# microsoft/StemGNN

Hardware: AMD Instinct MI355X
Metric: forecast-steps/sec (train) (higher is better)
Workload: dtype f32

## Files before the change

include/stemgnn_hip.h:

```cpp
#ifndef STEMGNN_HIP_H
#define STEMGNN_HIP_H

#include <stddef.h>
#include <stdint.h>

#ifdef __cplusplus
extern "C" {
#endif

#define SG_EINVAL (-10001)

#define SG_BLOCK_NPARAMS 33

const char* stemgnn_version(void);
int stemgnn_num_cus(void);

size_t stemgnn_table_floats(int W, int multi);
size_t stemgnn_packed_floats(int W, int multi);
size_t stemgnn_saved_floats(int B, int N, int W, int multi);
size_t stemgnn_scratch_floats(int B, int N, int W, int multi);
size_t stemgnn_gradpart_floats(int W, int multi, int nsplit);
size_t stemgnn_attn_saved_floats(int B, int N);
size_t stemgnn_attn_scratch_floats(int B, int N, int nchunk);
size_t stemgnn_scratch_offset_dG(int B, int N, int W, int multi);
// ... 58 lines not shown
int stemgnn_gru_bwd_overlap_ok(int B, int S, int Hd, int W);
size_t stemgnn_gru_bwd_ctl_words(int S);
int stemgnn_gru_bwd_rank2_begin(const float* dkey, const float* dquery, const float* wk, const float* wq, const float* x,
                                const float* w_hh, const float* h_ext, const float* reserve, int B, int S, int Hd, int W,
                                float* scratch, float* dw_ih, float* dw_hh, float* db_ih, float* db_hh, int* status,
                                unsigned* ctl, void* stream);
int stemgnn_gru_bwd_rank2_finish(const float* dkey, const float* dquery, const float* wk, const float* wq, const float* x,
                                 const float* w_hh, const float* h_ext, const float* reserve, int B, int S, int Hd, int W,
                                 float* scratch, float* dw_ih, float* dw_hh, float* db_ih, float* db_hh, int* status,
                                 unsigned* ctl, void* side_stream, void* stream);
int stemgnn_gru_bwd_recur(const float* dh_all, const float* x, const float* w_hh, const float* h_ext, const float* reserve,
                          int B, int S, int Hd, int W, float* scratch, int* status, void* stream);
int stemgnn_gru_bwd_rank2_recur(const float* dkey, float* dquery, int nchunk, const float* wk, const float* wq, const float* x,
                                const float* w_hh, const float* h_ext, const float* reserve, int B, int S, int Hd, int W,
                                float* scratch, int* status, void* stream);
int stemgnn_gru_input_grad(const float* scratch, const float* w_ih, int B, int S, int Hd, int W, float* dx, void* stream);

int stemgnn_block_pack(const float* const* params_host, const float* tables, float* packed,
                       int W, int multi, void* stream);
int stemgnn_block_pack_panels(const float* const* params_host, const float* tables, float* packed, int W, int multi,
                              void* stream);
int stemgnn_glu_fused_repack(float* packed, int W, int multi, void* stream);
int stemgnn_block_unpack_grads(const float* gradpart, int nsplit, const float* tables,
                               float* const* grads_host, int W, int multi, int has_backcast, void* stream);

int stemgnn_gft_fwd(const float* mul_L, const float* X, long xs_b, long xs_n, long xs_t,
                    float* G, int B, int N, int W, void* stream);
int stemgnn_gft_bwd(const float* mul_L, const float* X, long xs_b, long xs_n, long xs_t,
                    const float* dG, float* dX, float* dmul_L, int accumulate,
                    int B, int N, int W, void* stream);
int stemgnn_gft_bwd_dt2(const float* X0, long xs0_b, long xs0_n, long xs0_t, const float* dG0, const float* X1, long xs1_b,
                        long xs1_n, long xs1_t, const float* dG1, float* dmul_L, int B, int N, int W, void* stream);

int stemgnn_spectral_glu_fwd(const float* packed, float* saved, int B, int N, int W, int multi, void* stream);
int stemgnn_spectral_glu_bwd(const float* packed, const float* saved, float* scratch, float* gradpart,
                             int nsplit, int parts, int B, int N, int W, int multi, void* stream);
size_t stemgnn_glu_split_floats(int W, int multi, int splits);
int stemgnn_glu_split_panels(const float* packed, float* split, int W, int multi, int splits, void* stream);
int stemgnn_spectral_glu_fwd_split(const float* packed, const float* split, float* saved, int B, int N, int W, int multi,
                                   int splits, void* stream);
size_t stemgnn_glu_warm_saved_floats(int W, int multi);
int stemgnn_spectral_glu_fwd_warm(const float* packed, const float* split, float* saved, int B, int N, int W, int multi,
                                  int splits, void* stream);
int stemgnn_spectral_glu_dgrad_split(const float* packed, const float* split, const float* saved, float* scratch,
                                     int B, int N, int W, int multi, int splits, void* stream);
int stemgnn_glu_fused_bf16_ok(int W, int multi, int splits);

int stemgnn_igft_heads_fwd(const float* const* params_host, const float* packed, float* saved,
                           const float* X, long xs_b, long xs_n, long xs_t,
                           float* forecast, int accumulate, float* backcast,
                           int B, int N, int W, int multi, void* stream);
int stemgnn_igft_heads_bwd(const float* const* params_host, const float* packed, const float* saved,
                           const float* X, long xs_b, long xs_n, long xs_t,
                           const float* dforecast, const float* dbackcast, const float* backcast,
                           float* scratch, float* gradpart, int nsplit, int parts,
                           int B, int N, int W, int multi, void* stream);

int stemgnn_shortcut_dx(const float* scratch, const float* bs_w, float* dX, int B, int N, int W, int multi, void* stream);

int stemgnn_block_wgrad(const float* const* params_host, const float* packed, const float* saved,
                        const float* X, long xs_b, long xs_n, long xs_t, const float* dforecast, int has_bc,
                        float* scratch, float* gradpart, int nsplit, int cu_percent,
                        int B, int N, int W, int multi, void* stream);
int stemgnn_block_wgrad_split(const float* const* params_host, const float* packed, const float* saved,
                              const float* X, long xs_b, long xs_n, long xs_t, const float* dforecast, int has_bc,
                              float* scratch, float* gradpart, int nsplit, int cu_percent, int B, int N, int W,
// ... 74 lines not shown
```

stemgnn_amd/_lib.py:

```python
import ctypes
import os
from ctypes import POINTER, c_char_p, c_float, c_int, c_long, c_size_t, c_void_p

_HERE = os.path.dirname(os.path.abspath(__file__))
LIB_PATH = os.environ.get("STEMGNN_HIP_LIB", os.path.join(_HERE, "libstemgnn_hip.so"))
SG_BLOCK_NPARAMS = 33
SG_EINVAL = -10001
SG_PATH = {"glu_fwd_fused": 1, "glu_dgrad_fused": 2, "heads_fwd_fused": 4, "heads_bwd_fused": 8, "heads_bwd_16w": 16,
           "long_k": 32, "wgrad_fused": 64, "glu_wgrad_fused": 128}

_P = c_void_p
_PP = POINTER(c_void_p)

SIGNATURES = {
    "stemgnn_version": (c_char_p, []),
    "stemgnn_num_cus": (c_int, []),
    "stemgnn_table_floats": (c_size_t, [c_int, c_int]),
    "stemgnn_packed_floats": (c_size_t, [c_int, c_int]),
    "stemgnn_saved_floats": (c_size_t, [c_int, c_int, c_int, c_int]),
    "stemgnn_scratch_floats": (c_size_t, [c_int, c_int, c_int, c_int]),
    "stemgnn_scratch_offset_dG": (c_size_t, [c_int, c_int, c_int, c_int]),
    "stemgnn_gradpart_floats": (c_size_t, [c_int, c_int, c_int]),
    "stemgnn_attn_saved_floats": (c_size_t, [c_int, c_int]),
    "stemgnn_attn_scratch_floats": (c_size_t, [c_int, c_int, c_int]),
# ... 39 lines not shown
    "stemgnn_keyquery_wgrad": (c_int, [_P, _P, _P, _P, c_int, c_int, _P]),
    "stemgnn_attn_dquery_reduce": (c_int, [_P, c_int, c_int, c_int, _P, _P]),
    "stemgnn_keyquery_wgrad2": (c_int, [_P, _P, _P, _P, _P, c_int, c_int, _P]),
    "stemgnn_fc_tail_supported": (c_int, [c_int, c_int]),
    "stemgnn_fc_tail_scratch_floats": (c_size_t, [c_int, c_int, c_int, c_int]),
    "stemgnn_fc_tail_fwd": (c_int, [_P, _P, _P, _P, _P, c_int, c_int, c_int, c_int, _P, _P]),
    "stemgnn_fc_tail_bwd": (c_int, [_P, _P, _P, _P, _P, c_int, c_int, c_int, c_int, _P, _P, _P, _P, _P, _P, _P]),
    "stemgnn_fill_zero": (c_int, [_P, c_size_t, _P]),
    "stemgnn_rmsprop_step": (c_int, [_P, _P, _P, c_size_t, _P, c_float, c_float, c_int, c_float, _P]),
    "stemgnn_adam_step": (c_int, [_P, _P, _P, _P, c_size_t, _P, _P, c_float, c_float, c_float, c_int, c_float, _P]),
    "stemgnn_normalize_series": (c_int, [_P, _P, _P, c_int, _P, c_long, c_int, _P]),
    "stemgnn_window_gather": (c_int, [_P, _P, _P, _P, c_int, c_int, c_int, c_int, c_long, _P, _P]),
    "stemgnn_window_gather_queue": (c_int, [_P, _P, _P, _P, _P, c_int, c_int, c_int, c_int, c_long, _P, _P]),
    "stemgnn_mse_scratch_floats": (c_size_t, []),
    "stemgnn_mse_fwd": (c_int, [_P, _P, c_size_t, _P, _P, _P, _P]),
    "stemgnn_mse_bwd": (c_int, [_P, _P, c_size_t, _P, _P, _P]),
    "stemgnn_roll_window": (c_int, [_P, _P, _P, _P, c_int, c_int, c_int, c_int, c_int, c_int, _P]),
    "stemgnn_forecast_store": (c_int, [_P, _P, _P, _P, _P, c_int, c_int, c_int, c_long, _P]),
    "stemgnn_eval_scratch_doubles": (c_size_t, [c_long, c_int, c_int]),
    "stemgnn_eval_out_doubles": (c_size_t, [c_int, c_int]),
    "stemgnn_eval_metrics": (c_int, [_P, _P, _P, _P, c_long, c_int, c_int, _P, _P, _P]),
    "stemgnn_block_pack": (c_int, [_PP, _P, _P, c_int, c_int, _P]),
    "stemgnn_block_pack_panels": (c_int, [_PP, _P, _P, c_int, c_int, _P]),
    "stemgnn_block_unpack_grads": (c_int, [_P, c_int, _P, _PP, c_int, c_int, c_int, _P]),
    "stemgnn_gft_fwd": (c_int, [_P, _P, c_long, c_long, c_long, _P, c_int, c_int, c_int, _P]),
    "stemgnn_gft_bwd": (c_int, [_P, _P, c_long, c_long, c_long, _P, _P, _P, c_int, c_int, c_int, c_int, _P]),
    "stemgnn_gft_bwd_dt2": (c_int, [_P, c_long, c_long, c_long, _P, _P, c_long, c_long, c_long, _P, _P, c_int, c_int, c_int, _P]),
    "stemgnn_spectral_glu_fwd": (c_int, [_P, _P, c_int, c_int, c_int, c_int, _P]),
    "stemgnn_spectral_glu_bwd": (c_int, [_P, _P, _P, _P, c_int, c_int, c_int, c_int, c_int, c_int, _P]),
    "stemgnn_glu_split_floats": (c_size_t, [c_int, c_int, c_int]),
    "stemgnn_glu_split_panels": (c_int, [_P, _P, c_int, c_int, c_int, _P]),
    "stemgnn_glu_fused_bf16_ok": (c_int, [c_int, c_int, c_int]),
    "stemgnn_block_paths": (c_int, [c_int, c_int, c_int, c_int, c_int]),
    "stemgnn_spectral_glu_fwd_split": (c_int, [_P, _P, _P, c_int, c_int, c_int, c_int, c_int, _P]),
    "stemgnn_glu_warm_saved_floats": (c_size_t, [c_int, c_int]),
    "stemgnn_spectral_glu_fwd_warm": (c_int, [_P, _P, _P, c_int, c_int, c_int, c_int, c_int, _P]),
    "stemgnn_spectral_glu_dgrad_split": (c_int, [_P, _P, _P, _P, c_int, c_int, c_int, c_int, c_int, _P]),
    "stemgnn_igft_heads_fwd": (c_int, [_PP, _P, _P, _P, c_long, c_long, c_long, _P, c_int, _P,
                                       c_int, c_int, c_int, c_int, _P]),
    "stemgnn_igft_heads_bwd": (c_int, [_PP, _P, _P, _P, c_long, c_long, c_long, _P, _P, _P, _P, _P, c_int, c_int,
                                       c_int, c_int, c_int, c_int, _P]),
    "stemgnn_fc_tail_train_scratch_floats": (c_size_t, [c_int, c_int, c_int, c_int]),
    "stemgnn_fc_tail_train": (c_int, [_P, _P, _P, _P, _P, _P, c_int, c_int, c_int, c_int, _P, _P, _P, _P, _P, _P, _P, _P,
                                      _P, _P]),
    "stemgnn_fc_tail_train_rows": (c_int, [_P, _P, _P, _P, _P, _P, c_int, c_int, c_int, c_int, _P, _P, _P, _P]),
    "stemgnn_fc_tail_train_finish": (c_int, [_P, c_int, c_int, c_int, c_int, _P, _P, _P, _P, _P, _P, _P]),
    "stemgnn_infer_workspace_floats": (c_size_t, [c_int, c_int, c_int, c_int]),
    "stemgnn_infer_workspace_split_floats": (c_size_t, [c_int, c_int, c_int, c_int, c_int]),
    "stemgnn_gru_fwd_infer": (c_int, [_P, _P, _P, _P, _P, c_int, c_int, c_int, c_int, _P, _P, _P, _P]),
    "stemgnn_spectral_glu_fwd_infer": (c_int, [_P, _P, c_size_t, c_int, c_int, c_int, c_int, _P]),
    "stemgnn_spectral_glu_fwd_split_infer": (c_int, [_P, _P, _P, c_size_t, c_int, c_int, c_int, c_int, c_int, _P]),
    "stemgnn_igft_heads_fwd_infer": (c_int, [_PP, _P, _P, c_size_t, _P, c_long, c_long, c_long, _P, c_int, _P,
                                             c_int, c_int, c_int, c_int, _P]),
    "stemgnn_block_wgrad": (c_int, [_PP, _P, _P, _P, c_long, c_long, c_long, _P, c_int, _P, _P, c_int, c_int,
                                    c_int, c_int, c_int, c_int, _P]),
    "stemgnn_block_wgrad_split": (c_int, [_PP, _P, _P, _P, c_long, c_long, c_long, _P, c_int, _P, _P, c_int, c_int,
                                          c_int, c_int, c_int, c_int, c_int, _P]),
}

_lib = None


class StemGNNHipError(RuntimeError):
    pass


# ... 30 lines not shown
```

stemgnn_amd/csrc/block.hip:

```cpp
#include <hip/hip_runtime.h>

#include "../../include/stemgnn_hip.h"
#include "devattr.h"
#include "gemm2.h"
#include "gemm2s.h"
#include "gemm_core.h"
#include "layout.h"
#include "reduce.h"
#include "wgrad.h"
#include "heads.h"
#include "glu_fused.h"
#include "glu_fused_bf16.h"

#define SG_TRY(e)                                \
  do {                                           \
    hipError_t _e = (e);                         \
    if (_e != hipSuccess) return -(int)_e;       \
  } while (0)

__device__ __forceinline__ float sg_sigmoid(float v) { return __frcp_rn(1.f + __expf(-v)); }

struct SgDiv {
  unsigned d, magic;
  __device__ __forceinline__ int div(int x) const { return d == 1u ? x : (int)__umulhi((unsigned)x, magic); }
// ... 414 lines not shown
    const int w = z / S;
    const int n = nb[w];
    const int kb = k / rdiv[w], kr = k - kb * rdiv[w];
    const float v = pb[w][kb * sb[w] + kr * sn[w] + (j < n ? j : n - 1) * st[w]];
    return j < n ? v : 1.f;
  }
  __device__ void epi(int z, int i, int j, float v) const {
    const int w = z / S, s = z - w * S;
    part[w][((size_t)s * Mw[w] + i) * ldp[w] + j] = v;
  }
};

constexpr int SG_LONG_K = 640;
constexpr int SG_WG_MAX_TILES = 256;
static inline bool wg_tiles_fit(WgGemm* q, int n) { return wg_tile_index(q, n) <= SG_WG_MAX_TILES; }
static inline int split_chunk(int M, int S) { return ((M + S - 1) / S + 15) & ~15; }

extern "C" int stemgnn_gft_fwd(const float* mul_L, const float* X, long xs_b, long xs_n, long xs_t,
                               float* G, int B, int N, int W, void* stream) {
  if (!mul_L || !X || !G || B <= 0 || N <= 0 || W <= 0) return SG_EINVAL;
  if (!sg_div_ok(3L * N + 64, N) || !sg_div_ok((long)B * W + 64, W)) return SG_EINVAL;
  GftFwdOp op{mul_L + (size_t)N * N, XView{X, xs_b, xs_n, xs_t, N}, G, B, N, W, sg_div(N), sg_div(W)};
  hipStream_t st = (hipStream_t)stream;
  if (N <= 512) {
    if (xs_n == 1) SG_TRY((sg_launch_gemm<GftFwdOp, 32, 32, true, true, false, 128, true>(op, 3 * N, B * W, 1, st)));
    else SG_TRY((sg_launch_gemm<GftFwdOp, 32, 32, true, false, false, 128, true>(op, 3 * N, B * W, 1, st)));
    return 0;
  }
  if (xs_n == 1) SG_TRY((sg_launch_gemm<GftFwdOp, 32, 64, true, true, false, 64, true>(op, 3 * N, B * W, 1, st)));
  else SG_TRY((sg_launch_gemm<GftFwdOp, 32, 64, true, false, false, 64, true>(op, 3 * N, B * W, 1, st)));
  return 0;
}

extern "C" int stemgnn_gft_bwd(const float* mul_L, const float* X, long xs_b, long xs_n, long xs_t,
                               const float* dG, float* dX, float* dmul_L, int accumulate,
                               int B, int N, int W, void* stream) {
  if (!mul_L || !X || !dG || (!dmul_L && !dX) || B <= 0 || N <= 0 || W <= 0) return SG_EINVAL;
  hipStream_t st = (hipStream_t)stream;
  const bool bk128 = N <= 512;
  if (!sg_div_ok(3L * N + 128, N) || !sg_div_ok((long)B * W + 128, W)) return SG_EINVAL;
  if (dX) {
    GftBwdDxOp op{mul_L + (size_t)N * N, dG, dX, B, N, W, (size_t)B * N * 3 * W, sg_div(N), sg_div(W)};
    if (bk128) SG_TRY((sg_launch_gemm<GftBwdDxOp, 32, 32, false, false, false, 128, true>(op, N, B * W, 1, st)));
    else SG_TRY((sg_launch_gemm<GftBwdDxOp, 32, 32, false, false, false, 64, true>(op, N, B * W, 1, st)));
  }
  if (!dmul_L) return 0;
  GftBwdDtOp op{dG, XView{X, xs_b, xs_n, xs_t, N}, dmul_L + (size_t)N * N, B, N, W, accumulate, (size_t)B * N * 3 * W, sg_div(N),
                sg_div(W)};
  if (bk128) {
    if (xs_t == 1) SG_TRY((sg_launch_gemm<GftBwdDtOp, 32, 32, true, true, false, 128, true>(op, 3 * N, N, 1, st)));
    else SG_TRY((sg_launch_gemm<GftBwdDtOp, 32, 32, true, false, false, 128, true>(op, 3 * N, N, 1, st)));
    return 0;
  }
  if (xs_t == 1) SG_TRY((sg_launch_gemm<GftBwdDtOp, 32, 32, true, true, false, 64, true>(op, 3 * N, N, 1, st)));
  else SG_TRY((sg_launch_gemm<GftBwdDtOp, 32, 32, true, false, false, 64, true>(op, 3 * N, N, 1, st)));
  return 0;
}

extern "C" int stemgnn_gft_bwd_dt2(const float* X0, long xs0_b, long xs0_n, long xs0_t, const float* dG0, const float* X1,
                                   long xs1_b, long xs1_n, long xs1_t, const float* dG1, float* dmul_L, int B, int N, int W,
                                   void* stream) {
  if (!X0 || !dG0 || !X1 || !dG1 || !dmul_L || B <= 0 || N <= 0 || W <= 0) return SG_EINVAL;
  hipStream_t st = (hipStream_t)stream;
  if (!sg_div_ok(3L * N + 128, N) || !sg_div_ok(2L * B * W + 128, W)) return SG_EINVAL;
  GftBwdDt2Op op{{dG0, dG1}, {XView{X0, xs0_b, xs0_n, xs0_t, N}, XView{X1, xs1_b, xs1_n, xs1_t, N}}, dmul_L + (size_t)N * N,
                 B, N, W, (size_t)B * N * 3 * W, sg_div(N), sg_div(W)};
  if (N <= 512) SG_TRY((sg_launch_gemm<GftBwdDt2Op, 32, 32, true, false, false, 128, true>(op, 3 * N, N, 1, st)));
  else SG_TRY((sg_launch_gemm<GftBwdDt2Op, 32, 32, true, false, false, 64, true>(op, 3 * N, N, 1, st)));
  return 0;
}

struct GluFwdBufs {
  const float* G;
  float* out[2][3];
  float* gate[2][3];
};
static GluFwdBufs glu_bufs_saved(const SgDims& d, float* saved) {
  const SgSavedLayout S = sg_saved_layout(d);
  GluFwdBufs b;
  b.G = saved + S.G;
  for (int r = 0; r < 2; ++r)
    for (int l = 0; l < 3; ++l) { b.out[r][l] = saved + S.out[r][l]; b.gate[r][l] = saved + S.gate[r][l]; }
  return b;
}
static GluFwdBufs glu_bufs_infer(const SgDims& d, float* ws, bool pp) {
  const SgInferLayout I = sg_infer_layout(d, pp);
  GluFwdBufs b;
  b.G = ws + I.G;
  for (int r = 0; r < 2; ++r) {
    b.out[r][0] = pp ? ws + I.pp[r][0] : nullptr;
    b.out[r][1] = pp ? ws + I.pp[r][1] : nullptr;
    b.out[r][2] = ws + I.out2[r];
    for (int l = 0; l < 3; ++l) b.gate[r][l] = nullptr;
  }
  return b;
}
template <bool INF>
static int glu_fwd_layers(const SgDims& d, const float* packed, const unsigned short* const* fpl, int splits,
                          const GluFwdBufs& bf, hipStream_t st) {
  const SgPackedLayout P = sg_packed_layout(d);
  using Epi = GluFwdEpiT<!INF>;
  for (int l = 0; l < 3; ++l) {
// ... 837 lines not shown
```

stemgnn_amd/csrc/front.hip:

```cpp
#include <hip/hip_runtime.h>
#include <stdlib.h>
#include <stdint.h>

#include "../../include/stemgnn_hip.h"
#include "dq_reduce.h"
#include "gemm_core.h"
#include "layout.h"

#define SG_TRY(e)                                \
  do {                                           \
    hipError_t _e = (e);                         \
    if (_e != hipSuccess) return -(int)_e;       \
  } while (0)

constexpr int ATTN_NBC = 8;

__device__ __forceinline__ void sg_philox4(uint64_t seed, uint64_t offset, uint64_t idx, uint32_t (&w)[4]) {
  uint32_t c0 = (uint32_t)idx, c1 = (uint32_t)(idx >> 32), c2 = (uint32_t)offset, c3 = (uint32_t)(offset >> 32);
  uint32_t k0 = (uint32_t)seed, k1 = (uint32_t)(seed >> 32);
#pragma unroll
  for (int r = 0; r < 10; ++r) {
    const uint32_t hi0 = __umulhi(0xD2511F53u, c0), lo0 = 0xD2511F53u * c0;
    const uint32_t hi1 = __umulhi(0xCD9E8D57u, c2), lo1 = 0xCD9E8D57u * c2;
    c0 = hi1 ^ c1 ^ k0; c1 = lo1; c2 = hi0 ^ c3 ^ k1; c3 = lo0;
// ... 691 lines not shown
  if (!seed || !used || seed == used) return SG_EINVAL;
  hipLaunchKernelGGL(sg_dropout_seed_next_kernel, dim3(1), dim3(64), 0, (hipStream_t)stream, seed, used);
  SG_TRY(hipGetLastError());
  return 0;
}

extern "C" int stemgnn_dropout_mask(float drop_p, const uint64_t* seed, int B, int N, float* mask, void* stream) {
  if (!seed || !mask || B <= 0 || N <= 0) return SG_EINVAL;
  const size_t n = (size_t)B * N * N;
  hipLaunchKernelGGL(sg_dropout_mask_kernel, dim3((unsigned)((n + 255) / 256)), dim3(256), 0, (hipStream_t)stream,
                     drop_p, seed, n, N, mask);
  SG_TRY(hipGetLastError());
  return 0;
}

extern "C" int stemgnn_cheb_fwd(float* mul_L, int N, void* stream) {
  if (!mul_L || N <= 0) return SG_EINVAL;
  hipStream_t st = (hipStream_t)stream;
  const size_t nn = (size_t)N * N;
  float* L = mul_L + nn;
  ChebFwdOp op2{L, L, mul_L + 2 * nn, N, 0};
  if (N <= 512) {
    SG_TRY((sg_launch_gemm<ChebFwdOp, 32, 32, true, false, false, 128, true>(op2, N, N, 1, st)));
    ChebFwdOp op3b{L, mul_L + 2 * nn, mul_L + 3 * nn, N, 1};
    SG_TRY((sg_launch_gemm<ChebFwdOp, 32, 32, true, false, false, 128, true>(op3b, N, N, 1, st)));
    return 0;
  }
  SG_TRY((sg_launch_gemm<ChebFwdOp, 32, 32, true, false, false, 64, true>(op2, N, N, 1, st)));
  ChebFwdOp op3{L, mul_L + 2 * nn, mul_L + 3 * nn, N, 1};
  SG_TRY((sg_launch_gemm<ChebFwdOp, 32, 32, true, false, false, 64, true>(op3, N, N, 1, st)));
  return 0;
}

extern "C" int stemgnn_cheb_bwd(const float* mul_L, const float* dmul_L, float* dL, float* scratch, int N,
                                void* stream) {
  if (!mul_L || !dmul_L || !dL || !scratch || N <= 0) return SG_EINVAL;
  hipStream_t st = (hipStream_t)stream;
  const size_t nn = (size_t)N * N;
  float* dLp = scratch;
  float* dT2p = scratch + nn;
  ChebBwd1Op op1{mul_L + nn, mul_L + 2 * nn, dmul_L + nn, dmul_L + 2 * nn, dmul_L + 3 * nn, dLp, dT2p, N};
  if (N <= 512) {
    SG_TRY((sg_launch_gemm<ChebBwd1Op, 32, 32, true, true, false, 128, true>(op1, N, N, 2, st)));
    ChebBwd2Op op2b{mul_L + nn, dT2p, dLp, dL, N};
    SG_TRY((sg_launch_gemm<ChebBwd2Op, 32, 32, true, true, false, 128, true>(op2b, N, N, 1, st)));
    return 0;
  }
  SG_TRY((sg_launch_gemm<ChebBwd1Op, 32, 32, true, true, false, 64, true>(op1, N, N, 2, st)));
  ChebBwd2Op op2{mul_L + nn, dT2p, dLp, dL, N};
  SG_TRY((sg_launch_gemm<ChebBwd2Op, 32, 32, true, true, false, 64, true>(op2, N, N, 1, st)));
  return 0;
}
```

stemgnn_amd/csrc/gemm_core.h:

```cpp
#pragma once
#include <hip/hip_runtime.h>

typedef float sg_f32x4 __attribute__((ext_vector_type(4)));
#ifndef SG_CHAIN_PRIO
#define SG_CHAIN_PRIO 3
#endif

template <class Op, int BM, int BN, bool A_KFAST, bool B_KFAST, bool PAIR, int BK = 16, bool TWO_LEVEL = false>
__global__ __launch_bounds__(256) void sg_gemm_f32(const Op op) {
  static_assert(BK % 16 == 0, "BK");
  constexpr int TM = BM / 32;
  constexpr int TN = BN / 32;
  constexpr int SA = BM + (A_KFAST ? 17 : 16);
  constexpr int SB = BN + (B_KFAST ? 17 : 16);
  constexpr int RA = BM * BK / 256;
  constexpr int RB = BN * BK / 256;
  static_assert(BM % 32 == 0 && BN % 32 == 0, "tile");
  static_assert(!PAIR || (TN % 2 == 0), "PAIR needs an even number of 16-col tiles per wave");

  __builtin_amdgcn_s_setprio(SG_CHAIN_PRIO);
  __shared__ float lds[BK * SA + BK * SB];
  float* As = lds;
  float* Bs = lds + BK * SA;

  const int z = blockIdx.z;
  int M, N, K0, K1;
  if (!op.setup(z, M, N, K0, K1)) return;
  const int m0 = blockIdx.x * BM;
  const int n0 = blockIdx.y * BN;
  if (m0 >= M || n0 >= N) return;

  const int tid = threadIdx.x;
  const int lane = tid & 63;
  const int wave = tid >> 6;
// ... 91 lines not shown
  }

#pragma unroll
  for (int i = 0; i < TM; ++i) {
#pragma unroll
    for (int reg = 0; reg < 4; ++reg) {
      const int gi = m0 + wm * (BM / 2) + i * 16 + fk * 4 + reg;
      if (gi >= M) continue;
      if constexpr (PAIR) {
#pragma unroll
        for (int j = 0; j < TN; j += 2) {
          const int q0 = n0 + wn * (BN / 2) + j * 16;
          const int c = (q0 >> 1) + fi;
          if (q0 < N) op.epi2(z, gi, c, acc[i][j][reg], acc[i][j + 1][reg]);
        }
      } else {
#pragma unroll
        for (int j = 0; j < TN; ++j) {
          const int gj = n0 + wn * (BN / 2) + j * 16 + fi;
          if (gj < N) op.epi(z, gi, gj, acc[i][j][reg]);
        }
      }
    }
  }
}

template <class Op, int BM, int BN, bool A_KFAST, bool B_KFAST, bool PAIR, int BK = 16, bool TWO_LEVEL = false>
static inline hipError_t sg_launch_gemm(const Op& op, int maxM, int maxN, int nz, hipStream_t stream) {
  dim3 grid((maxM + BM - 1) / BM, (maxN + BN - 1) / BN, nz);
  if (grid.x == 0 || grid.y == 0 || grid.z == 0) return hipSuccess;
  hipLaunchKernelGGL((sg_gemm_f32<Op, BM, BN, A_KFAST, B_KFAST, PAIR, BK, TWO_LEVEL>), grid, dim3(256), 0, stream, op);
  return hipGetLastError();
}
```

stemgnn_amd/ops.py:

```python
import os
import weakref

import torch

from . import _lib

_NSPLIT = 32
_side_streams = {}


def _side_stream(device, index=0):
    key = (str(device), index)
    st = _side_streams.get(key)
    if st is None:
        st = torch.cuda.Stream(device=device)
        _side_streams[key] = st
    return st


def fresh_side_stream(device, index=0):
    _side_streams.pop((str(device), index), None)
    return _side_stream(device, index)


class HotPathState:

    def __init__(self):
        self.direct = False
        self.overlap = False
        self.prepacked = None
        self.preseed = None
        self.fork_event = None
        self.pending = None
        self.exact_group = None
        self.gru_front_live = False
        self.dh_factors = None
        self.block_grads_hook = None
        self.gru_ctl = None
        self.gru_ctl_zeroed = False
        self.warm_saved = None
        self.tail_finish = None
        self.side_probe = None
        _states.add(self)

    def set(self, direct=True, overlap=False):
        self.direct = bool(direct)
        self.overlap = bool(direct) and bool(overlap)
        return self

    def join(self):
        item, self.pending = self.pending, None
        if item is not None:
            side, keep = item
            torch.cuda.current_stream().wait_stream(side)
            del keep

    def reset(self):
        for item in (self.prepacked, self.pending):
            if item is not None:
                try:
                    (item[1] if item is self.prepacked else item[0]).synchronize()
                except RuntimeError:
                    pass
        self.prepacked = None
        self.preseed = None
        self.fork_event = None
        self.pending = None
        self.dh_factors = None
        self.gru_ctl_zeroed = False
        self.tail_finish = None


_states = weakref.WeakSet()
_NO_STATE = None
# ... 15 lines not shown


def _all_reduce_mean(t, group_world):
    group, world = group_world[0], group_world[1]
    fn = group_world[2] if len(group_world) > 2 else None
    if fn is not None:
        fn(t)
    else:
        import torch.distributed as dist
        dist.all_reduce(t, op=dist.ReduceOp.SUM, group=group)
    t.div_(world)


def set_direct_grad(model, flag=True, overlap=False):
    return model.hot_state.set(flag, overlap)


_NCHUNK = 16


def _wg_cu(which, B, N):
    if which == 0:
        return 90
    if N > 512:
        return 50
    lib = _lib.load()
    cus = lib.stemgnn_num_cus()
    busy = lib.stemgnn_gru_bwd_cus(B, N)
    return max(10, min(100, (cus - busy) * 100 // cus))


def _stream():
    return torch.cuda.current_stream().cuda_stream


def glu_splits():
    v = os.environ.get("STEMGNN_DTYPE", "f32").lower()
    if v in ("f32", "fp32", ""):
        return 0
    if v == "bf16x3":
        return 3
    if v == "bf16x2":
        return 2
    raise _lib.StemGNNHipError(f"STEMGNN_DTYPE={v!r}: expected f32, bf16x3 or bf16x2")


def _pack_block(lib, parr, tables, pk, W, multi, splits, stream):
    if splits:
        _lib.check(lib.stemgnn_block_pack_panels(parr, tables.data_ptr(), pk.data_ptr(), W, multi, stream), "block_pack_panels")
    else:
        _lib.check(lib.stemgnn_block_pack(parr, tables.data_ptr(), pk.data_ptr(), W, multi, stream), "block_pack")


def _split_panels(lib, pk, W, multi, splits, device, stream):
    sp = torch.empty(lib.stemgnn_glu_split_floats(W, multi, splits), device=device, dtype=torch.float32)
    _lib.check(lib.stemgnn_glu_split_panels(pk.data_ptr(), sp.data_ptr(), W, multi, splits, stream), "glu_split_panels")
    return sp


def _require_gpu(t, name):
    if not t.is_cuda:
        raise _lib.StemGNNHipError(
            f"{name} is on {t.device}: stemgnn_amd runs only on a HIP device (no CPU fallback)")
    if t.dtype != torch.float32:
        raise _lib.StemGNNHipError(f"{name} must be float32, got {t.dtype}")

# ... 593 lines not shown
            has_bc = s == 0
            garr = _lib.ptr_array(grads[s])
            keep.append((parr, garr))

            def heads(stream):
                _lib.check(lib.stemgnn_igft_heads_bwd(
                    parr, packed[s].data_ptr(), saved[s].data_ptr(), X.data_ptr(), sb, sn, stt, dfsum.data_ptr(),
                    dbackcast.data_ptr() if has_bc else None, backcast.data_ptr() if has_bc else None,
                    scratch.data_ptr(), gradpart.data_ptr(), nsplit, 1, B, N, W, multi, stream), "igft_heads_bwd")

            def glu(stream):
                if splits:
                    _lib.check(lib.stemgnn_spectral_glu_dgrad_split(
                        packed[s].data_ptr(), split[s].data_ptr(), saved[s].data_ptr(), scratch.data_ptr(),
                        B, N, W, multi, splits, stream), "spectral_glu_dgrad_split")
                    return
                _lib.check(lib.stemgnn_spectral_glu_bwd(
                    packed[s].data_ptr(), saved[s].data_ptr(), scratch.data_ptr(), gradpart.data_ptr(), nsplit, 1,
                    B, N, W, multi, stream), "spectral_glu_bwd")

            def wgrad(stream, cu_percent):
                _lib.check(lib.stemgnn_block_wgrad_split(
                    parr, packed[s].data_ptr(), saved[s].data_ptr(), X.data_ptr(), sb, sn, stt, dfsum.data_ptr(),
                    int(has_bc), scratch.data_ptr(), gradpart.data_ptr(), nsplit, cu_percent, B, N, W, multi,
                    2 if splits == 2 and os.environ.get("STEMGNN_WGRAD_BF16", "1") != "0" else 0, stream), "block_wgrad")

            def unpack(stream):
                _lib.check(lib.stemgnn_block_unpack_grads(
                    gradpart.data_ptr(), nsplit, tables.data_ptr(), garr, W, multi, int(has_bc), stream),
                    "block_unpack_grads")

            return heads, glu, wgrad, unpack

        dt1 = None
        for s in (1, 0):
            scratch = bufs[s][0]
            dG = scratch[off_dG:]
            X, sb, sn, stt = xviews[s]
            heads, glu, wgrad, unpack = stage_fns(s)
            heads(st)
            glu(st)
            if not overlap:
                if live[s]:
                    wgrad(st, 100)
                    unpack(st)
                _lib.check(lib.stemgnn_gft_bwd(
                    mul_L.data_ptr(), X.data_ptr(), sb, sn, stt, dG.data_ptr(),
                    dbackcast.data_ptr() if s == 1 else None, dmul_L.data_ptr(), int(s == 0), B, N, W, st), "gft_bwd")
            elif s == 1:
                _lib.check(lib.stemgnn_gft_bwd(mul_L.data_ptr(), X.data_ptr(), sb, sn, stt, dG.data_ptr(),
                                               dbackcast.data_ptr(), None, 0, B, N, W, st), "gft_bwd dX")
                dt1 = (X, sb, sn, stt, dG)
            else:
                fork = torch.cuda.Event()
                fork.record(main)
                X1, sb1, sn1, stt1, dG1 = dt1
                _lib.check(lib.stemgnn_gft_bwd_dt2(X.data_ptr(), sb, sn, stt, dG.data_ptr(), X1.data_ptr(), sb1, sn1, stt1,
                                                   dG1.data_ptr(), dmul_L.data_ptr(), B, N, W, st), "gft_bwd_dt2")
                side.wait_event(fork)
                with torch.cuda.stream(side):
                    sst = side.cuda_stream
                    for ss in (0, 1):
                        if not live[ss]:
                            continue
                        _h, _g, w2, u2 = (heads, glu, wgrad, unpack) if ss == 0 else stage_fns(1)
                        w2(sst, _wg_cu(ss, B, N))
                        u2(sst)
                        if state.side_probe is not None:
                            state.side_probe.append(lambda stream, w2=w2, pc=_wg_cu(ss, B, N): w2(stream, pc))
                            state.side_probe.append(u2)
                    if tail_finish is not None:
                        tail_finish(sst)
                        keep.append(tail_finish)
                        if state.side_probe is not None:
                            state.side_probe.append(tail_finish)
                    if state.block_grads_hook is not None:
                        state.block_grads_hook()
                keep.append(bufs)
        dX0 = None
        if nig[1]:
            X, sb, sn, stt = xviews[0]
            dX0 = torch.empty(B, N, W, device=dev, dtype=f32)
            _lib.check(lib.stemgnn_gft_bwd(mul_L.data_ptr(), X.data_ptr(), sb, sn, stt, scratch0[off_dG:].data_ptr(),
                                           dX0.data_ptr(), None, 0, B, N, W, st), "gft_bwd dX")
            _lib.check(lib.stemgnn_shortcut_dx(scratch0.data_ptr(), blocks[0][7].data_ptr(), dX0.data_ptr(), B, N, W, multi, st),
                       "shortcut_dx")
        if overlap:
            state.pending = (side, (keep, packed, saved, split, backcast, dfsum, dbackcast))
        dL = torch.empty(N, N, device=dev, dtype=f32)
        cheb_scratch = torch.empty(2 * N * N, device=dev, dtype=f32)
        _lib.check(lib.stemgnn_cheb_bwd(mul_L.data_ptr(), dmul_L.data_ptr(), dL.data_ptr(), cheb_scratch.data_ptr(),
                                        N, st), "cheb_bwd")
        factored = ctx.factored and ctx.needs_input_grad[0] and bool(lib.stemgnn_gru_bwd_rank2_ok(B, N))
        dh = torch.empty(1, device=dev, dtype=f32).expand(N, B, N) if factored else torch.empty_like(h)
        kq_direct = kq_live and state.direct and wk.grad is not None and wq.grad is not None
        if kq_live:
            dwk = wk.grad if kq_direct else torch.empty_like(wk)
            dwq = wq.grad if kq_direct else torch.empty_like(wq)
        elif factored:
            dwk = dwq = None
        else:
            dwk, dwq = torch.empty(2, N, device=dev, dtype=f32)
        _ptr = lambda t: None if t is None else t.data_ptr()
        attn_scratch = torch.empty(lib.stemgnn_attn_scratch_floats(B, N, _NCHUNK), device=dev, dtype=f32)
        use_drop = training and drop_p > 0.0
        exact = state.exact_group
        follower = bool(overlap and ctx.factored and state.gru_ctl_zeroed and lib.stemgnn_gru_bwd_overlap_ok(B, N, N, W))
        dq_parts = bool(factored and overlap and kq_direct and not follower)
        if not kq_live:
            dq_parts = bool(factored and not follower)
        for part in ((3,) if exact is None else (1, 2)):
            _lib.check(lib.stemgnn_attn_laplacian_bwd(
                dL.data_ptr(), h.data_ptr(), wk.data_ptr(), wq.data_ptr(), alpha, drop_p, int(training),
                seed.data_ptr() if use_drop else None, B, N, attn_saved.data_ptr(), attn_scratch.data_ptr(), _NCHUNK,
                None if factored else dh.data_ptr(), _ptr(dwk), _ptr(dwq),
                part | ((4 | (8 if dq_parts else 0)) if factored and part != 1 else 0), st), "attn_laplacian_bwd")
            if exact is not None and part == 1:
                _all_reduce_mean(attn_scratch[:N * N], exact)
        if factored:
            after = None
            if overlap and kq_direct:
                kq_ready = torch.cuda.Event()
                kq_ready.record(main)
                pend, hh, kdwk, kdwq = state.pending, h, dwk, dwq
                dq2 = torch.empty(B, N, device=dev, dtype=f32) if dq_parts else None
# ... 256 lines not shown
```

Measured before the change: 84620.

## Add split-K GEMM with workspace for graph backward products

```diff
diff --git a/include/stemgnn_hip.h b/include/stemgnn_hip.h
--- a/include/stemgnn_hip.h
+++ b/include/stemgnn_hip.h
@@ -114,6 +114,23 @@
 int stemgnn_gft_bwd_dt2(const float* X0, long xs0_b, long xs0_n, long xs0_t, const float* dG0, const float* X1, long xs1_b,
                         long xs1_n, long xs1_t, const float* dG1, float* dmul_L, int B, int N, int W, void* stream);
 
+#define SG_GP_GFT_DX  0
+#define SG_GP_GFT_DT  1
+#define SG_GP_GFT_DT2 2
+#define SG_GP_CHEB1   3
+#define SG_GP_CHEB2   4
+size_t stemgnn_graph_ws_floats(int B, int N, int W);
+int stemgnn_graph_splitk(int product, int B, int N, int W);
+int stemgnn_graph_ktiles(int product, int B, int N, int W);
+int stemgnn_gft_bwd_ws(const float* mul_L, const float* X, long xs_b, long xs_n, long xs_t,
+                       const float* dG, float* dX, float* dmul_L, int accumulate,
+                       int B, int N, int W, float* ws, int splitk, void* stream);
+int stemgnn_gft_bwd_dt2_ws(const float* X0, long xs0_b, long xs0_n, long xs0_t, const float* dG0, const float* X1, long xs1_b,
+                           long xs1_n, long xs1_t, const float* dG1, float* dmul_L, int B, int N, int W, float* ws, int splitk,
+                           void* stream);
+int stemgnn_cheb_bwd_ws(const float* mul_L, const float* dmul_L, float* dL, float* scratch, int B, int N, int W, float* ws,
+                        int splitk, void* stream);
+
 int stemgnn_spectral_glu_fwd(const float* packed, float* saved, int B, int N, int W, int multi, void* stream);
 int stemgnn_spectral_glu_bwd(const float* packed, const float* saved, float* scratch, float* gradpart,
                              int nsplit, int parts, int B, int N, int W, int multi, void* stream);
diff --git a/stemgnn_amd/_lib.py b/stemgnn_amd/_lib.py
--- a/stemgnn_amd/_lib.py
+++ b/stemgnn_amd/_lib.py
@@ -95,6 +95,13 @@
     "stemgnn_glu_split_panels": (c_int, [_P, _P, c_int, c_int, c_int, _P]),
     "stemgnn_glu_fused_bf16_ok": (c_int, [c_int, c_int, c_int]),
     "stemgnn_block_paths": (c_int, [c_int, c_int, c_int, c_int, c_int]),
+    "stemgnn_graph_ws_floats": (c_size_t, [c_int, c_int, c_int]),
+    "stemgnn_graph_splitk": (c_int, [c_int, c_int, c_int, c_int]),
+    "stemgnn_graph_ktiles": (c_int, [c_int, c_int, c_int, c_int]),
+    "stemgnn_gft_bwd_ws": (c_int, [_P, _P, c_long, c_long, c_long, _P, _P, _P, c_int, c_int, c_int, c_int, _P, c_int, _P]),
+    "stemgnn_gft_bwd_dt2_ws": (c_int, [_P, c_long, c_long, c_long, _P, _P, c_long, c_long, c_long, _P, _P, c_int, c_int, c_int,
+                                       _P, c_int, _P]),
+    "stemgnn_cheb_bwd_ws": (c_int, [_P, _P, _P, _P, c_int, c_int, c_int, _P, c_int, _P]),
     "stemgnn_spectral_glu_fwd_split": (c_int, [_P, _P, _P, c_int, c_int, c_int, c_int, c_int, _P]),
     "stemgnn_glu_warm_saved_floats": (c_size_t, [c_int, c_int]),
     "stemgnn_spectral_glu_fwd_warm": (c_int, [_P, _P, _P, c_int, c_int, c_int, c_int, c_int, _P]),
diff --git a/stemgnn_amd/csrc/block.hip b/stemgnn_amd/csrc/block.hip
--- a/stemgnn_amd/csrc/block.hip
+++ b/stemgnn_amd/csrc/block.hip
@@ -470,21 +470,32 @@
   return 0;
 }
 
-extern "C" int stemgnn_gft_bwd(const float* mul_L, const float* X, long xs_b, long xs_n, long xs_t,
-                               const float* dG, float* dX, float* dmul_L, int accumulate,
-                               int B, int N, int W, void* stream) {
+static int gft_bwd_impl(const float* mul_L, const float* X, long xs_b, long xs_n, long xs_t, const float* dG, float* dX,
+                        float* dmul_L, int accumulate, int B, int N, int W, float* ws, int splitk, void* stream) {
   if (!mul_L || !X || !dG || (!dmul_L && !dX) || B <= 0 || N <= 0 || W <= 0) return SG_EINVAL;
   hipStream_t st = (hipStream_t)stream;
   const bool bk128 = N <= 512;
   if (!sg_div_ok(3L * N + 128, N) || !sg_div_ok((long)B * W + 128, W)) return SG_EINVAL;
+  const SgSkGeom gx = sg_graph_geom(SG_GP_GFT_DX, B, N, W), gt = sg_graph_geom(SG_GP_GFT_DT, B, N, W);
+  const int top = std::max(dX ? sg_splitk_top(gx) : 1, dmul_L ? sg_splitk_top(gt) : 1);
+  if (splitk > top) return SG_EINVAL;
+  const int sx = ws ? sg_splitk_resolve(SG_GP_GFT_DX, gx, splitk) : 1;
+  const int stt = ws ? sg_splitk_resolve(SG_GP_GFT_DT, gt, splitk) : 1;
   if (dX) {
     GftBwdDxOp op{mul_L + (size_t)N * N, dG, dX, B, N, W, (size_t)B * N * 3 * W, sg_div(N), sg_div(W)};
-    if (bk128) SG_TRY((sg_launch_gemm<GftBwdDxOp, 32, 32, false, false, false, 128, true>(op, N, B * W, 1, st)));
+    if (sx > 1) SG_TRY((sg_launch_gemm_splitk<GftBwdDxOp, false, false>(op, gx, sx, ws + sg_graph_region(SG_GP_GFT_DX, B, N, W), st)));
+    else if (bk128) SG_TRY((sg_launch_gemm<GftBwdDxOp, 32, 32, false, false, false, 128, true>(op, N, B * W, 1, st)));
     else SG_TRY((sg_launch_gemm<GftBwdDxOp, 32, 32, false, false, false, 64, true>(op, N, B * W, 1, st)));
   }
   if (!dmul_L) return 0;
   GftBwdDtOp op{dG, XView{X, xs_b, xs_n, xs_t, N}, dmul_L + (size_t)N * N, B, N, W, accumulate, (size_t)B * N * 3 * W, sg_div(N),
                 sg_div(W)};
+  if (stt > 1) {
+    float* region = ws + sg_graph_region(SG_GP_GFT_DT, B, N, W);
+    if (xs_t == 1) SG_TRY((sg_launch_gemm_splitk<GftBwdDtOp, true, true>(op, gt, stt, region, st)));
+    else SG_TRY((sg_launch_gemm_splitk<GftBwdDtOp, true, false>(op, gt, stt, region, st)));
+    return 0;
+  }
   if (bk128) {
     if (xs_t == 1) SG_TRY((sg_launch_gemm<GftBwdDtOp, 32, 32, true, true, false, 128, true>(op, 3 * N, N, 1, st)));
     else SG_TRY((sg_launch_gemm<GftBwdDtOp, 32, 32, true, false, false, 128, true>(op, 3 * N, N, 1, st)));
@@ -495,17 +506,60 @@
   return 0;
 }
 
+extern "C" int stemgnn_gft_bwd(const float* mul_L, const float* X, long xs_b, long xs_n, long xs_t,
+                               const float* dG, float* dX, float* dmul_L, int accumulate,
+                               int B, int N, int W, void* stream) {
+  return gft_bwd_impl(mul_L, X, xs_b, xs_n, xs_t, dG, dX, dmul_L, accumulate, B, N, W, nullptr, 1, stream);
+}
+static inline bool sg_ws_ok(const float* ws, int splitk) { return splitk >= 0 && (ws ? ((uintptr_t)ws & 15) == 0 : splitk == 1); }
+extern "C" int stemgnn_gft_bwd_ws(const float* mul_L, const float* X, long xs_b, long xs_n, long xs_t,
+                                  const float* dG, float* dX, float* dmul_L, int accumulate,
+                                  int B, int N, int W, float* ws, int splitk, void* stream) {
+  if (!sg_ws_ok(ws, splitk)) return SG_EINVAL;
+  return gft_bwd_impl(mul_L, X, xs_b, xs_n, xs_t, dG, dX, dmul_L, accumulate, B, N, W, ws, splitk, stream);
+}
+
+static int gft_bwd_dt2_impl(const float* X0, long xs0_b, long xs0_n, long xs0_t, const float* dG0, const float* X1, long xs1_b,
+                            long xs1_n, long xs1_t, const float* dG1, float* dmul_L, int B, int N, int W, float* ws, int splitk,
+                            void* stream) {
+  if (!X0 || !dG0 || !X1 || !dG1 || !dmul_L || B <= 0 || N <= 0 || W <= 0) return SG_EINVAL;
+  hipStream_t st = (hipStream_t)stream;
+  if (!sg_div_ok(3L * N + 128, N) || !sg_div_ok(2L * B * W + 128, W)) return SG_EINVAL;
+  const SgSkGeom g = sg_graph_geom(SG_GP_GFT_DT2, B, N, W);
+  if (splitk > sg_splitk_top(g)) return SG_EINVAL;
+  const int S = ws ? sg_splitk_resolve(SG_GP_GFT_DT2, g, splitk) : 1;
+  GftBwdDt2Op op{{dG0, dG1}, {XView{X0, xs0_b, xs0_n, xs0_t, N}, XView{X1, xs1_b, xs1_n, xs1_t, N}}, dmul_L + (size_t)N * N,
+                 B, N, W, (size_t)B * N * 3 * W, sg_div(N), sg_div(W)};
+  if (S > 1) SG_TRY((sg_launch_gemm_splitk<GftBwdDt2Op, true, false>(op, g, S, ws + sg_graph_region(SG_GP_GFT_DT2, B, N, W), st)));
+  else if (N <= 512) SG_TRY((sg_launch_gemm<GftBwdDt2Op, 32, 32, true, false, false, 128, true>(op, 3 * N, N, 1, st)));
+  else SG_TRY((sg_launch_gemm<GftBwdDt2Op, 32, 32, true, false, false, 64, true>(op, 3 * N, N, 1, st)));
+  return 0;
+}
 extern "C" int stemgnn_gft_bwd_dt2(const float* X0, long xs0_b, long xs0_n, long xs0_t, const float* dG0, const float* X1,
                                    long xs1_b, long xs1_n, long xs1_t, const float* dG1, float* dmul_L, int B, int N, int W,
                                    void* stream) {
-  if (!X0 || !dG0 || !X1 || !dG1 || !dmul_L || B <= 0 || N <= 0 || W <= 0) return SG_EINVAL;
-  hipStream_t st = (hipStream_t)stream;
-  if (!sg_div_ok(3L * N + 128, N) || !sg_div_ok(2L * B * W + 128, W)) return SG_EINVAL;
-  GftBwdDt2Op op{{dG0, dG1}, {XView{X0, xs0_b, xs0_n, xs0_t, N}, XView{X1, xs1_b, xs1_n, xs1_t, N}}, dmul_L + (size_t)N * N,
-                 B, N, W, (size_t)B * N * 3 * W, sg_div(N), sg_div(W)};
-  if (N <= 512) SG_TRY((sg_launch_gemm<GftBwdDt2Op, 32, 32, true, false, false, 128, true>(op, 3 * N, N, 1, st)));
-  else SG_TRY((sg_launch_gemm<GftBwdDt2Op, 32, 32, true, false, false, 64, true>(op, 3 * N, N, 1, st)));
-  return 0;
+  return gft_bwd_dt2_impl(X0, xs0_b, xs0_n, xs0_t, dG0, X1, xs1_b, xs1_n, xs1_t, dG1, dmul_L, B, N, W, nullptr, 1, stream);
+}
+extern "C" int stemgnn_gft_bwd_dt2_ws(const float* X0, long xs0_b, long xs0_n, long xs0_t, const float* dG0, const float* X1,
+                                      long xs1_b, long xs1_n, long xs1_t, const float* dG1, float* dmul_L, int B, int N, int W,
+                                      float* ws, int splitk, void* stream) {
+  if (!sg_ws_ok(ws, splitk)) return SG_EINVAL;
+  return gft_bwd_dt2_impl(X0, xs0_b, xs0_n, xs0_t, dG0, X1, xs1_b, xs1_n, xs1_t, dG1, dmul_L, B, N, W, ws, splitk, stream);
+}
+
+extern "C" size_t stemgnn_graph_ws_floats(int B, int N, int W) {
+  if (B <= 0 || N <= 0 || W <= 0) return 0;
+  const size_t n = sg_graph_region(SG_GP_COUNT, B, N, W);
+  return n ? n : 64;
+}
+extern "C" int stemgnn_graph_splitk(int product, int B, int N, int W) {
+  if (product < 0 || product >= SG_GP_COUNT || B <= 0 || N <= 0 || W <= 0) return SG_EINVAL;
+  return sg_splitk_choice(product, sg_graph_geom(product, B, N, W));
+}
+extern "C" int stemgnn_graph_ktiles(int product, int B, int N, int W) {
+  if (product < 0 || product >= SG_GP_COUNT || B <= 0 || N <= 0 || W <= 0) return SG_EINVAL;
+  const SgSkGeom g = sg_graph_geom(product, B, N, W);
+  return g.splittable ? g.T : 1;
 }
 
 struct GluFwdBufs {
diff --git a/stemgnn_amd/csrc/front.hip b/stemgnn_amd/csrc/front.hip
--- a/stemgnn_amd/csrc/front.hip
+++ b/stemgnn_amd/csrc/front.hip
@@ -747,22 +747,32 @@
   return 0;
 }
 
-extern "C" int stemgnn_cheb_bwd(const float* mul_L, const float* dmul_L, float* dL, float* scratch, int N,
-                                void* stream) {
+static int cheb_bwd_impl(const float* mul_L, const float* dmul_L, float* dL, float* scratch, int N, float* ws, int splitk,
+                         void* stream) {
   if (!mul_L || !dmul_L || !dL || !scratch || N <= 0) return SG_EINVAL;
   hipStream_t st = (hipStream_t)stream;
   const size_t nn = (size_t)N * N;
   float* dLp = scratch;
   float* dT2p = scratch + nn;
+  const SgSkGeom g1 = sg_graph_geom(SG_GP_CHEB1, 1, N, 1), g2 = sg_graph_geom(SG_GP_CHEB2, 1, N, 1);
+  if (splitk > sg_splitk_top(g2)) return SG_EINVAL;
+  const int s1 = ws ? sg_splitk_resolve(SG_GP_CHEB1, g1, splitk) : 1, s2 = ws ? sg_splitk_resolve(SG_GP_CHEB2, g2, splitk) : 1;
   ChebBwd1Op op1{mul_L + nn, mul_L + 2 * nn, dmul_L + nn, dmul_L + 2 * nn, dmul_L + 3 * nn, dLp, dT2p, N};
-  if (N <= 512) {
-    SG_TRY((sg_launch_gemm<ChebBwd1Op, 32, 32, true, true, false, 128, true>(op1, N, N, 2, st)));
-    ChebBwd2Op op2b{mul_L + nn, dT2p, dLp, dL, N};
-    SG_TRY((sg_launch_gemm<ChebBwd2Op, 32, 32, true, true, false, 128, true>(op2b, N, N, 1, st)));
-    return 0;
-  }
-  SG_TRY((sg_launch_gemm<ChebBwd1Op, 32, 32, true, true, false, 64, true>(op1, N, N, 2, st)));
   ChebBwd2Op op2{mul_L + nn, dT2p, dLp, dL, N};
-  SG_TRY((sg_launch_gemm<ChebBwd2Op, 32, 32, true, true, false, 64, true>(op2, N, N, 1, st)));
-  return 0;
-}
+  if (s1 > 1) SG_TRY((sg_launch_gemm_splitk<ChebBwd1Op, true, true>(op1, g1, s1, ws, st)));
+  else if (N <= 512) SG_TRY((sg_launch_gemm<ChebBwd1Op, 32, 32, true, true, false, 128, true>(op1, N, N, 2, st)));
+  else SG_TRY((sg_launch_gemm<ChebBwd1Op, 32, 32, true, true, false, 64, true>(op1, N, N, 2, st)));
+  if (s2 > 1) SG_TRY((sg_launch_gemm_splitk<ChebBwd2Op, true, true>(op2, g2, s2, ws + g1.floats, st)));
+  else if (N <= 512) SG_TRY((sg_launch_gemm<ChebBwd2Op, 32, 32, true, true, false, 128, true>(op2, N, N, 1, st)));
+  else SG_TRY((sg_launch_gemm<ChebBwd2Op, 32, 32, true, true, false, 64, true>(op2, N, N, 1, st)));
+  return 0;
+}
+extern "C" int stemgnn_cheb_bwd(const float* mul_L, const float* dmul_L, float* dL, float* scratch, int N,
+                                void* stream) {
+  return cheb_bwd_impl(mul_L, dmul_L, dL, scratch, N, nullptr, 1, stream);
+}
+extern "C" int stemgnn_cheb_bwd_ws(const float* mul_L, const float* dmul_L, float* dL, float* scratch, int B, int N, int W,
+                                   float* ws, int splitk, void* stream) {
+  if (B <= 0 || W <= 0 || N <= 0 || splitk < 0 || (ws ? ((uintptr_t)ws & 15) != 0 : splitk != 1)) return SG_EINVAL;
+  return cheb_bwd_impl(mul_L, dmul_L, dL, scratch, N, ws ? ws + sg_graph_region(SG_GP_CHEB1, B, N, W) : nullptr, splitk, stream);
+}
diff --git a/stemgnn_amd/csrc/gemm_core.h b/stemgnn_amd/csrc/gemm_core.h
--- a/stemgnn_amd/csrc/gemm_core.h
+++ b/stemgnn_amd/csrc/gemm_core.h
@@ -1,5 +1,7 @@
 #pragma once
 #include <hip/hip_runtime.h>
+
+#include "../../include/stemgnn_hip.h"
 
 typedef float sg_f32x4 __attribute__((ext_vector_type(4)));
 #ifndef SG_CHAIN_PRIO
@@ -157,3 +159,198 @@
   hipLaunchKernelGGL((sg_gemm_f32<Op, BM, BN, A_KFAST, B_KFAST, PAIR, BK, TWO_LEVEL>), grid, dim3(256), 0, stream, op);
   return hipGetLastError();
 }
+
+constexpr int SG_SK_BK = 128;
+constexpr int SG_SK_TILE = 32 * 32;
+constexpr int SG_SK_MAX_KT = 16;
+constexpr int SG_SK_CUS = 256;
+
+template <class Op, bool A_KFAST, bool B_KFAST>
+__global__ __launch_bounds__(256) void sg_gemm_f32_splitk(const Op op, float* __restrict__ part, unsigned* __restrict__ cnt,
+                                                          int S, int T, int gx, int gy, int ntiles, int ntp) {
+  constexpr int BM = 32, BN = 32, BK = SG_SK_BK;
+  constexpr int SA = BM + (A_KFAST ? 17 : 16);
+  constexpr int SB = BN + (B_KFAST ? 17 : 16);
+  constexpr int RA = BM * BK / 256;
+  constexpr int RB = BN * BK / 256;
+
+  __builtin_amdgcn_s_setprio(SG_CHAIN_PRIO);
+  __shared__ float lds[BK * SA + BK * SB];
+  float* As = lds;
+  float* Bs = lds + BK * SA;
+
+  const int slice = blockIdx.x / ntp;
+  const int tile = blockIdx.x - slice * ntp;
+  if (tile >= ntiles) return;
+  const int z = tile / (gx * gy);
+  const int rz = tile - z * gx * gy;
+  const int by = rz / gx, bx = rz - by * gx;
+  int M, N, K0, K1;
+  if (!op.setup(z, M, N, K0, K1)) return;
+  const int m0 = bx * BM;
+  const int n0 = by * BN;
+
+  const int kt_base = T / S, kt_rem = T - kt_base * S;
+  const int kt_lo = slice * kt_base + (slice < kt_rem ? slice : kt_rem);
+  const int kt_hi = kt_lo + kt_base + (slice < kt_rem ? 1 : 0);
+  const int nk0 = kt_base + (kt_rem > 0 ? 1 : 0);
+
+  const int tid = threadIdx.x;
+  const int lane = tid & 63;
+  const int wave = tid >> 6;
+  const int wm = wave >> 1, wn = wave & 1;
+
+  sg_f32x4 acc = (sg_f32x4){0.f, 0.f, 0.f, 0.f}, acc2 = (sg_f32x4){0.f, 0.f, 0.f, 0.f};
+  float ra[RA], rb[RB];
+
+  auto gload = [&](int kbase) {
+#pragma unroll
+    for (int r = 0; r < RA; ++r) {
+      const int e = tid + 256 * r;
+      const int k = A_KFAST ? (e % BK) : (e / BM);
+      const int i = A_KFAST ? (e / BK) : (e % BM);
+      const int gi = m0 + i, gk = kbase + k;
+      const float v = op.a(z, gi < M ? gi : M - 1, gk < K1 ? gk : K1 - 1);
+      ra[r] = (gi < M && gk < K1) ? v : 0.f;
+    }
+#pragma unroll
+    for (int r = 0; r < RB; ++r) {
+      const int e = tid + 256 * r;
+      const int k = B_KFAST ? (e % BK) : (e / BN);
+      const int j = B_KFAST ? (e / BK) : (e % BN);
+      const int gj = n0 + j, gk = kbase + k;
+      const float v = op.b(z, gk < K1 ? gk : K1 - 1, gj < N ? gj : N - 1);
+      rb[r] = (gj < N && gk < K1) ? v : 0.f;
+    }
+  };
+  auto lstore = [&]() {
+#pragma unroll
+    for (int r = 0; r < RA; ++r) {
+      const int e = tid + 256 * r;
+      const int k = A_KFAST ? (e % BK) : (e / BM);
+      const int i = A_KFAST ? (e / BK) : (e % BM);
+      As[k * SA + i] = ra[r];
+    }
+#pragma unroll
+    for (int r = 0; r < RB; ++r) {
+      const int e = tid + 256 * r;
+      const int k = B_KFAST ? (e % BK) : (e / BN);
+      const int j = B_KFAST ? (e / BK) : (e % BN);
+      Bs[k * SB + j] = rb[r];
+    }
+  };
+
+  const int fi = lane & 15;
+  const int fk = lane >> 4;
+  sg_f32x4* const ptile = reinterpret_cast<sg_f32x4*>(part + (size_t)tile * T * SG_SK_TILE) + tid;
+
+  gload(kt_lo * BK);
+  for (int kt = kt_lo; kt < kt_hi; ++kt) {
+    lstore();
+    __syncthreads();
+    if (kt + 1 < kt_hi) gload((kt + 1) * BK);
+#pragma unroll
+    for (int ks = 0; ks < BK; ks += 4) {
+      const float af = As[(ks + fk) * SA + wm * (BM / 2) + fi];
+      const float bf = Bs[(ks + fk) * SB + wn * (BN / 2) + fi];
+      acc = __builtin_amdgcn_mfma_f32_16x16x4f32(af, bf, acc, 0, 0, 0);
+    }
+    if (slice == 0) acc2 += acc;
+    else ptile[kt * 256] = acc;
+    acc = (sg_f32x4){0.f, 0.f, 0.f, 0.f};
+    __syncthreads();
+  }
+  if (slice == 0) ptile[0] = acc2;
+
+  asm volatile("s_waitcnt vmcnt(0)" ::: "memory");
+  __syncthreads();
+  if (tid == 0) {
+    __builtin_amdgcn_fence(__ATOMIC_RELEASE, "agent");
+    asm volatile("s_waitcnt vmcnt(0)" ::: "memory");
+    const unsigned ticket = __hip_atomic_fetch_add(cnt + tile, 1u, __ATOMIC_RELAXED, __HIP_MEMORY_SCOPE_AGENT);
+    const bool last = ticket == (unsigned)(S - 1);
+    if (last) {
+      __builtin_amdgcn_fence(__ATOMIC_ACQUIRE, "agent");
+      asm volatile("s_waitcnt vmcnt(0)" ::: "memory");
+    }
+    lds[0] = last ? 1.f : 0.f;
+  }
+  __syncthreads();
+  if (lds[0] == 0.f) return;
+
+  sg_f32x4 sum = ptile[0];
+  for (int s0 = nk0; s0 < T; s0 += 8) {
+    sg_f32x4 p[8];
+#pragma unroll
+    for (int i = 0; i < 8; ++i) p[i] = ptile[(s0 + i < T ? s0 + i : 0) * 256];
+#pragma unroll
+    for (int i = 0; i < 8; ++i)
+      if (s0 + i < T) sum += p[i];
+  }
+  if (tid == 0) __hip_atomic_store(cnt + tile, 0u, __ATOMIC_RELAXED, __HIP_MEMORY_SCOPE_AGENT);
+
+#pragma unroll
+  for (int reg = 0; reg < 4; ++reg) {
+    const int gi = m0 + wm * (BM / 2) + fk * 4 + reg;
+    const int gj = n0 + wn * (BN / 2) + fi;
+    if (gi < M && gj < N) op.epi(z, gi, gj, sum[reg]);
+  }
+}
+
+constexpr int SG_GP_COUNT = 5;
+
+struct SgSkGeom {
+  int gx, gy, nz, ntiles, T;
+  bool splittable;
+  size_t floats;
+};
+static inline SgSkGeom sg_graph_geom(int product, int B, int N, int W) {
+  long M = N, Nn = N, K = N;
+  int nz = 1;
+  const long BW = (long)B * W;
+  switch (product) {
+    case SG_GP_GFT_DX: M = N; Nn = BW; K = 3L * N; break;
+    case SG_GP_GFT_DT: M = 3L * N; Nn = N; K = BW; break;
+    case SG_GP_GFT_DT2: M = 3L * N; Nn = N; K = 2 * BW; break;
+    case SG_GP_CHEB1: nz = 2; break;
+    default: K = 2L * N; break;
+  }
+  SgSkGeom g;
+  g.gx = (int)((M + 31) / 32);
+  g.gy = (int)((Nn + 31) / 32);
+  g.nz = nz;
+  const long nt = (long)g.gx * g.gy * nz, T = (K + SG_SK_BK - 1) / SG_SK_BK;
+  g.ntiles = (int)nt;
+  g.T = T > (1 << 20) ? (1 << 20) : (int)T;
+  g.splittable = N <= 512 && T >= 2 && T <= SG_SK_MAX_KT && nt * SG_SK_MAX_KT < (1L << 24);
+  g.floats = g.splittable ? (size_t)nt * T * SG_SK_TILE + (size_t)((nt + 63) & ~63L) : 0;
+  return g;
+}
+static inline size_t sg_graph_region(int product, int B, int N, int W) {
+  size_t off = 0;
+  for (int p = 0; p < product; ++p) off += sg_graph_geom(p, B, N, W).floats;
+  return off;
+}
+constexpr int SG_SK_MAX_WGS = SG_SK_CUS + SG_SK_CUS / 4;
+static inline int sg_splitk_choice(int product, const SgSkGeom& g) {
+  (void)product;
+  if (!g.splittable) return 1;
+  const int S = SG_SK_MAX_WGS / g.ntiles;
+  return S < 1 ? 1 : (S > g.T ? g.T : S);
+}
+static inline int sg_splitk_top(const SgSkGeom& g) { return g.splittable ? g.T : 1; }
+static inline int sg_splitk_resolve(int product, const SgSkGeom& g, int splitk) {
+  if (splitk == 0) return sg_splitk_choice(product, g);
+  const int top = sg_splitk_top(g);
+  return splitk < top ? splitk : top;
+}
+
+template <class Op, bool A_KFAST, bool B_KFAST>
+static inline hipError_t sg_launch_gemm_splitk(const Op& op, const SgSkGeom& g, int S, float* region, hipStream_t stream) {
+  if (g.ntiles <= 0) return hipSuccess;
+  const int ntp = (g.ntiles + 7) & ~7;
+  unsigned* cnt = reinterpret_cast<unsigned*>(region + (size_t)g.ntiles * g.T * SG_SK_TILE);
+  hipLaunchKernelGGL((sg_gemm_f32_splitk<Op, A_KFAST, B_KFAST>), dim3((unsigned)(ntp * S)), dim3(256), 0, stream, op, region, cnt,
+                     S, g.T, g.gx, g.gy, g.ntiles, ntp);
+  return hipGetLastError();
+}
diff --git a/stemgnn_amd/ops.py b/stemgnn_amd/ops.py
--- a/stemgnn_amd/ops.py
+++ b/stemgnn_amd/ops.py
@@ -40,6 +40,7 @@
         self.gru_ctl_zeroed = False
         self.warm_saved = None
         self.tail_finish = None
+        self.graph_ws = None
         self.side_probe = None
         _states.add(self)
 
@@ -121,6 +122,19 @@
 
 def _stream():
     return torch.cuda.current_stream().cuda_stream
+
+
+def _graph_ws(state, lib, B, N, W, device):
+    key = (B, N, W, str(torch.device(device)))
+    if state.graph_ws is None:
+        state.graph_ws = {}
+    ws = state.graph_ws.get(key)
+    if ws is None:
+        n = lib.stemgnn_graph_ws_floats(B, N, W)
+        ws = torch.empty(n, device=device, dtype=torch.float32)
+        _lib.check(lib.stemgnn_fill_zero(ws.data_ptr(), 4 * n, _stream()), "fill_zero")
+        state.graph_ws[key] = ws
+    return ws.data_ptr()
 
 
 def glu_splits():
@@ -780,6 +794,8 @@
 
             return heads, glu, wgrad, unpack
 
+        gws = _graph_ws(state, lib, B, N, W, dev)
+        sk_beside = 1 if overlap else 0
         dt1 = None
         for s in (1, 0):
             scratch = bufs[s][0]
@@ -792,19 +808,20 @@
                 if live[s]:
                     wgrad(st, 100)
                     unpack(st)
-                _lib.check(lib.stemgnn_gft_bwd(
+                _lib.check(lib.stemgnn_gft_bwd_ws(
                     mul_L.data_ptr(), X.data_ptr(), sb, sn, stt, dG.data_ptr(),
-                    dbackcast.data_ptr() if s == 1 else None, dmul_L.data_ptr(), int(s == 0), B, N, W, st), "gft_bwd")
+                    dbackcast.data_ptr() if s == 1 else None, dmul_L.data_ptr(), int(s == 0), B, N, W, gws, 0, st), "gft_bwd")
             elif s == 1:
-                _lib.check(lib.stemgnn_gft_bwd(mul_L.data_ptr(), X.data_ptr(), sb, sn, stt, dG.data_ptr(),
-                                               dbackcast.data_ptr(), None, 0, B, N, W, st), "gft_bwd dX")
+                _lib.check(lib.stemgnn_gft_bwd_ws(mul_L.data_ptr(), X.data_ptr(), sb, sn, stt, dG.data_ptr(),
+                                                  dbackcast.data_ptr(), None, 0, B, N, W, gws, 0, st), "gft_bwd dX")
                 dt1 = (X, sb, sn, stt, dG)
             else:
                 fork = torch.cuda.Event()
                 fork.record(main)
                 X1, sb1, sn1, stt1, dG1 = dt1
-                _lib.check(lib.stemgnn_gft_bwd_dt2(X.data_ptr(), sb, sn, stt, dG.data_ptr(), X1.data_ptr(), sb1, sn1, stt1,
-                                                   dG1.data_ptr(), dmul_L.data_ptr(), B, N, W, st), "gft_bwd_dt2")
+                _lib.check(lib.stemgnn_gft_bwd_dt2_ws(X.data_ptr(), sb, sn, stt, dG.data_ptr(), X1.data_ptr(), sb1, sn1, stt1,
+                                                      dG1.data_ptr(), dmul_L.data_ptr(), B, N, W, gws, sk_beside, st),
+                           "gft_bwd_dt2")
                 side.wait_event(fork)
                 with torch.cuda.stream(side):
                     sst = side.cuda_stream
@@ -829,16 +846,16 @@
         if nig[1]:
             X, sb, sn, stt = xviews[0]
             dX0 = torch.empty(B, N, W, device=dev, dtype=f32)
-            _lib.check(lib.stemgnn_gft_bwd(mul_L.data_ptr(), X.data_ptr(), sb, sn, stt, scratch0[off_dG:].data_ptr(),
-                                           dX0.data_ptr(), None, 0, B, N, W, st), "gft_bwd dX")
+            _lib.check(lib.stemgnn_gft_bwd_ws(mul_L.data_ptr(), X.data_ptr(), sb, sn, stt, scratch0[off_dG:].data_ptr(),
+                                              dX0.data_ptr(), None, 0, B, N, W, gws, sk_beside, st), "gft_bwd dX")
             _lib.check(lib.stemgnn_shortcut_dx(scratch0.data_ptr(), blocks[0][7].data_ptr(), dX0.data_ptr(), B, N, W, multi, st),
                        "shortcut_dx")
         if overlap:
             state.pending = (side, (keep, packed, saved, split, backcast, dfsum, dbackcast))
         dL = torch.empty(N, N, device=dev, dtype=f32)
         cheb_scratch = torch.empty(2 * N * N, device=dev, dtype=f32)
-        _lib.check(lib.stemgnn_cheb_bwd(mul_L.data_ptr(), dmul_L.data_ptr(), dL.data_ptr(), cheb_scratch.data_ptr(),
-                                        N, st), "cheb_bwd")
+        _lib.check(lib.stemgnn_cheb_bwd_ws(mul_L.data_ptr(), dmul_L.data_ptr(), dL.data_ptr(), cheb_scratch.data_ptr(),
+                                           B, N, W, gws, sk_beside, st), "cheb_bwd")
         factored = ctx.factored and ctx.needs_input_grad[0] and bool(lib.stemgnn_gru_bwd_rank2_ok(B, N))
         dh = torch.empty(1, device=dev, dtype=f32).expand(N, B, N) if factored else torch.empty_like(h)
         kq_direct = kq_live and state.direct and wk.grad is not None and wq.grad is not None
```

New measurement: 84940 (median of 6 runs). No clear change (+0.4%).
